# AvalonEnjoyer/pytorch-ViT-paper-replication

Hardware: AMD Instinct MI355X
Metric: images/sec (whole node) ViT-B/16 224px bf16 at 1/2/4/8 MI355X (higher is better)
Workload: dtype bf16; 1 GPU; model=ViT-B/16, global_batch=256, per_gpu_batch=256, seq_len=197, image_size=224, parallelism=dp1, impl=fused, grad_transport=none, optimizer=Adam(wd=0.03 decay group) + clip 1.0 + warmup/linear-decay LR, dropout=0.1 (mlp, embedding)

## Files before the change

### pytorch_vit_paper_replication_amd/csrc/bindings.cpp

```cpp
#include <cstdlib>
#include <algorithm>
#include <map>
#include <torch/extension.h>
#include <c10/hip/HIPStream.h>
#include <hip/hip_runtime.h>

#include "kernels.h"

namespace {

hipStream_t stream() { return c10::hip::getCurrentHIPStream().stream(); }
using ScratchKey = std::pair<int, int64_t>;
ScratchKey scratch_key(int dev) { return std::make_pair(dev, (int64_t)c10::hip::getCurrentHIPStream().id()); }
template <class T>
std::map<ScratchKey, T>& scratch_map() {
  static auto* m = new std::map<ScratchKey, T>();
  return *m;
}
struct SkCounters { torch::Tensor t; };
struct DetWs { torch::Tensor t; };
struct DqWs { torch::Tensor t; };
struct AttnWs { torch::Tensor t; };

int num_cus() {
// ... 733 lines not shown
void attn_dbias_reduce(torch::Tensor part, int64_t B, int64_t H, torch::Tensor dbias) {
  TORCH_CHECK(dbias.is_cuda() && dbias.scalar_type() == torch::kFloat32 && dbias.is_contiguous() && dbias.numel() % (3 * H) == 0,
              "attn_dbias_reduce: f32 [3D] bias gradient");
  const int64_t DH = dbias.numel() / (3 * H);
  TORCH_CHECK(part.is_cuda() && part.scalar_type() == torch::kFloat32 && part.is_contiguous() && part.numel() % (B * H * 3 * DH) == 0,
              "attn_dbias_reduce: f32 [B*H][R][3 * head dim] partials");
  const int64_t NQ = part.numel() / (B * H * 3 * DH);
  auto ws = torch::empty({(int64_t)pvr_attn_dbias_splits((int)B, (int)NQ) * H * 2 * DH}, part.options());
  check(pvr_attn_dbias_reduce(part.data_ptr<float>(), ws.data_ptr<float>(), dbias.data_ptr<float>(), (int)B, (int)H, (int)NQ,
                              (int)(DH * H), stream()),
        "attn_dbias_reduce");
}

torch::Tensor dq_workspace(int64_t numel, const torch::TensorOptions& opts, bool drop = false) {
  DqWs& d = scratch_map<DqWs>()[scratch_key((int)opts.device().index())];
  if (drop) {
    d.t = torch::Tensor();
    return torch::Tensor();
  }
  if (!d.t.defined() || d.t.numel() < numel) d.t = torch::zeros({numel}, opts.dtype(torch::kFloat32));
  return d.t;
}

torch::Tensor attn_scratch(int64_t numel, const torch::TensorOptions& opts) {
  AttnWs& d = scratch_map<AttnWs>()[scratch_key((int)opts.device().index())];
  if (!d.t.defined() || d.t.numel() < numel) d.t = torch::empty({numel}, opts.dtype(torch::kFloat32));
  return d.t;
}

void free_scratch() {
  scratch_map<TailBufs>().clear();
  scratch_map<SkCounters>().clear();
  scratch_map<DetWs>().clear();
  scratch_map<DqWs>().clear();
  scratch_map<AttnWs>().clear();
}

int64_t attn_bwd_bias_rows(int64_t B, int64_t N, int64_t H, int64_t D, bool drop) {
  return pvr_attn_bwd_part_rows((int)B, (int)N, (int)H, (int)D, 3 * D, D, D, 3 * D, drop ? 1 : 0);
}

bool attn_bwd_q8_ok(int64_t B, int64_t N, int64_t H, int64_t D, bool drop) {
  return pvr_attn_bwd_q8_ok((int)N, drop ? 1 : 0) && !pvr_attn_bwd_uses_pipe((int)B, (int)N, (int)H, (int)D, 3 * D, D, D, 3 * D, drop ? 1 : 0);
}

torch::Tensor attn_bwd(torch::Tensor dout, torch::Tensor qkv, torch::Tensor out, torch::Tensor lse, int64_t B, int64_t N, int64_t H,
                       double scale, c10::optional<torch::Tensor> dbias, c10::optional<torch::Tensor> dbias_part_out,
                       c10::optional<torch::Tensor> seed, int64_t seed_offset, double drop_p, c10::optional<torch::Tensor> q_out,
                       c10::optional<torch::Tensor> q_scale, c10::optional<torch::Tensor> q_amax, bool q_only,
                       int64_t q_fmt) {
  const int64_t D = qkv.size(1) / 3;
  auto dqkv = torch::empty_like(qkv);
  torch::Tensor dq_acc;
  int dq_rezero = 0;
  const pvr::DropSite drop = drop_args(seed, seed_offset, drop_p, "attn_bwd");
  const int has_drop = drop.seed ? 1 : 0;
  const int64_t dh = D / H;
  torch::Tensor dbias_part, old_part;
  const bool want_db = dbias.has_value() && dbias->defined();
  const int64_t lds[4] = {ld_of(qkv, "qkv"), ld_of(dout, "dout"), ld_of(out, "out"), ld_of(dqkv, "dqkv")};
  const int prow = pvr_attn_bwd_part_rows((int)B, (int)N, (int)H, (int)D, lds[0], lds[1], lds[2], lds[3], has_drop);
  const bool parts = prow > 0;
  const bool pipe = pvr_attn_bwd_uses_pipe((int)B, (int)N, (int)H, (int)D, lds[0], lds[1], lds[2], lds[3], has_drop) != 0;
  const bool part_out = dbias_part_out.has_value() && dbias_part_out->defined();
  if (part_out) {
    TORCH_CHECK(parts && !want_db, "dbias_part: shapes with attn_bwd_bias_rows > 0 only, and not together with dbias");
    TORCH_CHECK(dbias_part_out->is_cuda() && dbias_part_out->scalar_type() == torch::kFloat32 && dbias_part_out->is_contiguous() &&
                    dbias_part_out->numel() == B * H * prow * 3 * dh,
                "dbias_part [B*H][attn_bwd_bias_rows][3 * head dim] f32");
    dbias_part = *dbias_part_out;
  }
  if (want_db) {
    TORCH_CHECK(dbias->numel() == 3 * D && dbias->scalar_type() == torch::kFloat32 && dbias->is_contiguous(), "dbias [3D] f32");
    if (parts)
      dbias_part = torch::empty({B * H, (int64_t)prow, 3 * dh}, qkv.options().dtype(torch::kFloat32));
    else if (2 * (dh / 16) <= 2 * pvr_attn_bwd_waves((int)N))
      old_part = torch::empty({B * pvr_attn_bwd_key_blocks((int)N), 3 * D}, qkv.options().dtype(torch::kFloat32));
  }
  const int old_db = old_part.defined() ? 1 : 0;
  if (pvr_attn_bwd_needs_dq_acc((int)N, (int)dh, old_db, has_drop, g_deterministic ? 1 : 0)) {
    dq_acc = dq_workspace(B * N * D, qkv.options());
    dq_rezero = dq_acc.defined() ? 1 : 0;
    if (!dq_acc.defined()) dq_acc = torch::zeros({B * N, D}, qkv.options().dtype(torch::kFloat32));
  }
  const pvr::Fp8Copy q8 = fp8_copy(q_out, q_scale, q_amax, q_fmt, B * N, 3 * D, 4, "attn_bwd");
  if (q8.out)
    TORCH_CHECK(pvr_attn_bwd_q8_ok((int)N, has_drop) && !old_db && !pipe, "attn_bwd: no e5m2 dQKV copy for this shape (see attn_bwd_q8_ok)");
  auto ws = attn_scratch(pvr_attn_bwd_ws_floats((int)B, (int)N, (int)H, (int)D, old_db, has_drop, g_deterministic ? 1 : 0), qkv.options());
  pvr::AttnBwdParams p{};
  p.qkv = bf(qkv, "qkv"); p.ld = lds[0];
  p.out = bf(out, "out"); p.ld_o = lds[2];
  p.dout = bf(dout, "dout"); p.ld_do = lds[1];
  p.dqkv = bf_mut(dqkv, "dqkv"); p.ld_dq = lds[3];
  p.lse = f32(lse, "lse"); p.ws = ws.data_ptr<float>();
  p.dq_acc = dq_acc.defined() ? dq_acc.data_ptr<float>() : nullptr; p.dq_rezero = dq_rezero;
  p.dbias = pipe && dbias_part.defined() ? dbias_part.data_ptr<float>() : old_db ? old_part.data_ptr<float>() : nullptr;
  p.bpart = !pipe && dbias_part.defined() ? dbias_part.data_ptr<float>() : nullptr;
  p.B = (int)B; p.N = (int)N; p.H = (int)H; p.D = (int)D; p.scale = (float)scale;
  p.drop = drop; p.q8 = q8; p.q8_only = q_only && q8.out ? 1 : 0;
  const hipError_t err = pvr_attn_bwd(&p, stream());
  if (err != hipSuccess && dq_rezero) dq_workspace(0, qkv.options(), true);
  check(err, "attn_bwd");
  if (want_db) {
    if (parts)
      attn_dbias_reduce(dbias_part, B, H, *dbias);
    else if (old_db)
      dbias->add_(old_part.sum(0));
    else
      dbias->add_(dqkv.sum(0, false, torch::kFloat32));
  }
  return dqkv;
}

}

extern "C" const char* pvr_src_hash(void);

PYBIND11_MODULE(TORCH_EXTENSION_NAME, m) {
  m.doc() = "MI355X (gfx950) HIP kernels for pytorch_vit_paper_replication_amd";
  m.def("source_hash", []() { return std::string(pvr_src_hash()); },
        "content hash of the csrc/ sources this binary was built from (build.source_hash())");
  m.def("gemm_tail_split", [](int64_t M, int64_t N, int64_t K, int64_t elem_bytes, int64_t max_units) {
    return pvr_gemm_tail_split((int)M, (int)N, (int)K, (int)elem_bytes, (int)max_units); },
    py::arg("M"), py::arg("N"), py::arg("K"), py::arg("elem_bytes"), py::arg("max_units") = 0,
    "K-parts of the split tail round this GEMM shape gets (0: none)");
  m.def("set_attn_dbg", [](torch::Tensor t) { pvr_set_attn_dbg(t.defined() && t.numel() ? t.data_ptr() : nullptr); },
        "diagnostic builds (-DPVR_ATTN_STAMPS): int64 buffer for the attention backward's phase stamps "
        "[workgroup * waves + wave][8] (scripts/attn_stamps.py); a no-op otherwise");
  m.def("set_attn_prep_xcd", &pvr_set_attn_prep_xcd, "attention backward pre-pass: XCD-contiguous (batch, head) pairs (1) or round-robin (0, default); A/B");
  m.def("set_ln_fwd_q8_grid", &pvr_set_ln_fwd_q8_grid, "LayerNorm forward with the e4m3 copy: grid cap in workgroups per CU (A/B)");
  m.def("set_attn_fwd_head_qf", &pvr_set_attn_fwd_head_qf, "whole-head attention forward (dh 64, N <= 256): 16-query fragments per wave (1 = default, 2 = half the LDS reads with 7 waves; A/B)");
  m.def("set_attn_fwd_qg", &pvr_set_attn_fwd_qg, "tiled attention forward: 16-query groups per wave (0 = auto by query padding, 1 = round-3 form, 2 = forced; A/B)");
  m.def("set_fp8_persistent", &pvr_set_fp8_persistent, "fp8 fwd/dgrad GEMMs on the persistent ping-pong: 1 when the epilogue has no per-row input (default), 0 never (A/B)");
  m.def("set_deterministic", &set_deterministic, "deterministic reductions (partial rows + ordered sum) instead of float atomics");
  m.def("deterministic", &deterministic);
  m.def("set_gemm_tail", &set_gemm_tail, "split-K tail of the last dispatch round on (True, default) / off (A/B)");
  m.def("gemm", &gemm,py::arg("A"), py::arg("a_kcontig"), py::arg("B"), py::arg("b_kcontig"), py::arg("C"),
        py::arg("M"), py::arg("N"), py::arg("K"), py::arg("epi"), py::arg("bias"), py::arg("resid"), py::arg("addend"),
        py::arg("addend_period"), py::arg("aux"), py::arg("row_group"), py::arg("row_stride_group"),
        py::arg("row_offset"), py::arg("seed"), py::arg("seed_offset"), py::arg("drop_p"), py::arg("k_split"),
        py::arg("tile_cfg"), py::arg("dbg") = py::none(), py::arg("colsum") = py::none(),
        py::arg("epi_staged") = 0, py::arg("tail_limit") = 0, py::arg("reduce_out") = py::none(), py::arg("reduce_acc") = true);
  m.def("splitk_timeouts", &splitk_timeouts, py::arg("like"), py::arg("reset") = false);
  m.def("num_cus", &num_cus);
  m.def("layernorm_fwd", &layernorm_fwd);
  m.def("free_scratch", &free_scratch);
  m.def("layernorm_fwd_q8", &layernorm_fwd_q8);
  m.def("layernorm_bwd", &layernorm_bwd, py::arg("dy"), py::arg("dy_stride"), py::arg("x"), py::arg("x_stride"),
        py::arg("mean"), py::arg("rstd"), py::arg("w"), py::arg("dres"), py::arg("dres_stride"), py::arg("dx"),
        py::arg("dx_stride"), py::arg("dw"), py::arg("db"), py::arg("rows"), py::arg("dsum") = py::none(),
        py::arg("dz") = py::none(), py::arg("seed") = py::none(), py::arg("seed_offset") = 0, py::arg("drop_p") = 0.0,
        py::arg("q_out") = py::none(), py::arg("q_scale") = py::none(), py::arg("q_amax") = py::none(),
        py::arg("dz_nostore") = false, py::arg("q_fmt") = 1);
  m.def("cast_f32_bf16", &cast_f32_bf16);
  m.def("splitk_epilogue", &splitk_epilogue);
  m.def("attn_bwd_bias_rows", &attn_bwd_bias_rows, py::arg("B"), py::arg("N"), py::arg("H"), py::arg("D"), py::arg("drop") = false);
  m.def("attn_dbias_reduce", &attn_dbias_reduce);
  m.def("splitk_reduce", &splitk_reduce);
  m.def("pad_cols_bf16", &pad_cols_bf16);
  m.def("transpose_batched", &transpose_batched);
  m.def("colsum", &colsum, py::arg("dy"), py::arg("rows"), py::arg("N"), py::arg("db"), py::arg("dz"), py::arg("seed"),
        py::arg("seed_offset"), py::arg("drop_p"), py::arg("q_out") = py::none(), py::arg("q_scale") = py::none(),
        py::arg("q_amax") = py::none(), py::arg("q_fmt") = 1);
  m.def("im2col", &im2col);
  m.def("im2col_u8", &im2col_u8, py::arg("img"), py::arg("out"), py::arg("mean"), py::arg("std"), py::arg("geom"), py::arg("H"),
        py::arg("W"), py::arg("P"), py::arg("Kp"));
  m.def("cls_rows", &cls_rows);
  m.def("patch_bwd", &patch_bwd);
  m.def("xent", &xent, py::arg("logits"), py::arg("labels"), py::arg("dlogits"), py::arg("correct"), py::arg("grad_scale"),
        py::arg("mean") = py::none());
  m.def("grad_norm", &grad_norm);
  m.def("norm_partial_blocks", []() { return pvr_norm_partial_blocks(); });
  m.def("adam", &adam);
  m.def("adam_t", &adam_t);
  m.def("scale_by_clip", &scale_by_clip);
  m.def("head_fwd", &head_fwd);
  m.def("head_bwd", &head_bwd, py::arg("dlogits"), py::arg("xhat"), py::arg("rstd"), py::arg("gamma"), py::arg("beta"), py::arg("W"),
        py::arg("B"), py::arg("N"), py::arg("dW") = py::none(), py::arg("db") = py::none(), py::arg("dgamma") = py::none(),
        py::arg("dbeta") = py::none());
  m.def("scale_by", &scale_by);
  m.def("metrics_accum", &metrics_accum);
  m.def("rng_next", &rng_next);
  m.def("zero_f32", &zero_f32);
  m.def("gemm_fp8", &gemm_fp8, py::arg("A"), py::arg("fmt_a"), py::arg("B"), py::arg("fmt_b"), py::arg("C"), py::arg("M"),
        py::arg("N"), py::arg("K"), py::arg("epi"), py::arg("scale_a"), py::arg("scale_b"), py::arg("bias") = py::none(),
        py::arg("resid") = py::none(), py::arg("aux") = py::none(), py::arg("seed") = py::none(), py::arg("seed_offset") = 0,
        py::arg("drop_p") = 0.0, py::arg("colsum") = py::none(), py::arg("q_out") = py::none(), py::arg("q_scale") = py::none(),
        py::arg("q_amax") = py::none(), py::arg("q_fmt") = 0, py::arg("c_skip") = false, py::arg("tail_limit") = 0);
  m.def("fp8_transpose", &fp8_transpose);
  m.def("gemm_fp8_wgrad_mn", &gemm_fp8_wgrad_mn, py::arg("dy8"), py::arg("x8"), py::arg("ws"), py::arg("N"), py::arg("K"),
        py::arg("T"), py::arg("scale_a"), py::arg("scale_b"), py::arg("ksplit"), py::arg("fmt_a") = 1);
  m.def("fp8_quant", &fp8_quant, py::arg("x"), py::arg("y"), py::arg("qscale"), py::arg("amax"), py::arg("fmt"));
  m.def("fp8_dequant", &fp8_dequant, py::arg("x"), py::arg("dscale") = py::none(), py::arg("fmt") = 0);
  m.def("fp8_scale_update", &fp8_scale_update);
  m.def("fp8_quant_t", &fp8_quant_t);
  m.def("gemm_fp8_wgrad", &gemm_fp8_wgrad, py::arg("A8"), py::arg("B8"), py::arg("ws"), py::arg("N"), py::arg("K"), py::arg("Tp"),
        py::arg("scale_a"), py::arg("scale_b"), py::arg("ksplit"), py::arg("fmt_a") = 1);
  m.def("fp8_quant_multi", &fp8_quant_multi, py::arg("segs"), py::arg("nchunks"), py::arg("qscale"), py::arg("amax"), py::arg("fmt"),
        py::arg("amax_only"));
  m.def("attn_fwd", &attn_fwd, py::arg("qkv"), py::arg("B"), py::arg("N"), py::arg("H"), py::arg("scale"),
        py::arg("seed") = py::none(), py::arg("seed_offset") = 0, py::arg("drop_p") = 0.0, py::arg("q_out") = py::none(),
        py::arg("q_scale") = py::none(), py::arg("q_amax") = py::none(), py::arg("q_only") = false);
  m.def("attn_bwd", &attn_bwd, py::arg("dout"), py::arg("qkv"), py::arg("out"), py::arg("lse"), py::arg("B"), py::arg("N"),
        py::arg("H"), py::arg("scale"), py::arg("dbias") = py::none(), py::arg("dbias_part") = py::none(),
        py::arg("seed") = py::none(), py::arg("seed_offset") = 0, py::arg("drop_p") = 0.0, py::arg("q_out") = py::none(),
        py::arg("q_scale") = py::none(), py::arg("q_amax") = py::none(), py::arg("q_only") = false,
        py::arg("q_fmt") = 1);
  m.def("attn_bwd_q8_ok", &attn_bwd_q8_ok, "attn_bwd can write dQKV's e5m2 copy for this shape");
  m.def("arch", []() { return std::string("gfx950"); });
}
```

### pytorch_vit_paper_replication_amd/csrc/layernorm.hip

```cpp
#include "common.h"
#include "kernels.h"

namespace pvr {
namespace {

template <int MAXCH>
__global__ void __launch_bounds__(256) ln_fwd_kernel(const uint16_t* __restrict__ x, int64_t x_stride,
                                                      const float* __restrict__ w, const float* __restrict__ b,
                                                      uint16_t* __restrict__ y, int64_t y_stride,
                                                      float* __restrict__ mean_out, float* __restrict__ rstd_out,
                                                      int rows, int D, float eps) {
  const int lane = threadIdx.x & 63;
  const int row = blockIdx.x * 4 + (threadIdx.x >> 6);
  if (row >= rows) return;
  const int nch = D >> 3;
  PVR_ASSERT((D & 7) == 0 && nch <= 64 * MAXCH);
  const uint16_t* xr = x + (int64_t)row * x_stride;
  float v[MAXCH][8];
  float s = 0.f;
#pragma unroll
  for (int i = 0; i < MAXCH; ++i) {
    const int c = lane + 64 * i;
    if (c < nch) {
      const uint4 q = *(const uint4*)(xr + c * 8);
      const uint32_t u[4] = {q.x, q.y, q.z, q.w};
#pragma unroll
      for (int j = 0; j < 4; ++j) {
        v[i][2 * j] = bf2f(u[j] & 0xFFFF);
        v[i][2 * j + 1] = bf2f(u[j] >> 16);
      }
#pragma unroll
      for (int j = 0; j < 8; ++j) s += v[i][j];
    } else {
#pragma unroll
      for (int j = 0; j < 8; ++j) v[i][j] = 0.f;
    }
  }
  const float mean = wave_sum(s) / D;
  float ss = 0.f;
#pragma unroll
  for (int i = 0; i < MAXCH; ++i) {
    const int c = lane + 64 * i;
    if (c < nch) {
#pragma unroll
      for (int j = 0; j < 8; ++j) {
        const float d = v[i][j] - mean;
        ss += d * d;
      }
    }
  }
  const float rstd = rsqrtf(wave_sum(ss) / D + eps);
  uint16_t* yr = y + (int64_t)row * y_stride;
#pragma unroll
  for (int i = 0; i < MAXCH; ++i) {
    const int c = lane + 64 * i;
    if (c < nch) {
      const float4 w0 = *(const float4*)(w + c * 8), w1 = *(const float4*)(w + c * 8 + 4);
      const float4 b0 = *(const float4*)(b + c * 8), b1 = *(const float4*)(b + c * 8 + 4);
      const float ww[8] = {w0.x, w0.y, w0.z, w0.w, w1.x, w1.y, w1.z, w1.w};
      const float bb[8] = {b0.x, b0.y, b0.z, b0.w, b1.x, b1.y, b1.z, b1.w};
      float o[8];
#pragma unroll
      for (int j = 0; j < 8; ++j) o[j] = (v[i][j] - mean) * rstd * ww[j] + bb[j];
      uint4 q;
      q.x = pack2bf(o[0], o[1]); q.y = pack2bf(o[2], o[3]);
      q.z = pack2bf(o[4], o[5]); q.w = pack2bf(o[6], o[7]);
      *(uint4*)(yr + c * 8) = q;
    }
  }
  if (lane == 0) {
    mean_out[row] = mean;
    rstd_out[row] = rstd;
  }
}

template <int MAXCH>
__global__ void __launch_bounds__(256) ln_fwd_q8_kernel(const uint16_t* __restrict__ x, int64_t x_stride,
                                                        const float* __restrict__ w, const float* __restrict__ b,
                                                        uint16_t* __restrict__ y, int64_t y_stride, uint8_t* __restrict__ yq,
                                                        int64_t q_stride, const float* __restrict__ qscale,
                                                        unsigned* __restrict__ amax, float* __restrict__ mean_out,
                                                        float* __restrict__ rstd_out, int rows, int D, float eps) {
  __shared__ float wm[4];
  const int lane = threadIdx.x & 63;
  const int nch = D >> 3;
  const float qs = *qscale;
  float am = 0.f;
  for (int row = blockIdx.x * 4 + (int)(threadIdx.x >> 6); row < rows; row += gridDim.x * 4) {
    const uint16_t* xr = x + (int64_t)row * x_stride;
    float v[MAXCH][8];
    float s = 0.f;
#pragma unroll
    for (int i = 0; i < MAXCH; ++i) {
      const int c = lane + 64 * i;
      if (c < nch) {
        const uint4 q = *(const uint4*)(xr + c * 8);
        const uint32_t u[4] = {q.x, q.y, q.z, q.w};
#pragma unroll
        for (int j = 0; j < 4; ++j) {
          v[i][2 * j] = bf2f(u[j] & 0xFFFF);
          v[i][2 * j + 1] = bf2f(u[j] >> 16);
        }
#pragma unroll
        for (int j = 0; j < 8; ++j) s += v[i][j];
      } else {
#pragma unroll
        for (int j = 0; j < 8; ++j) v[i][j] = 0.f;
      }
    }
    const float mean = wave_sum(s) / D;
    float ss = 0.f;
#pragma unroll
    for (int i = 0; i < MAXCH; ++i) {
      const int c = lane + 64 * i;
      if (c < nch) {
#pragma unroll
        for (int j = 0; j < 8; ++j) {
          const float d = v[i][j] - mean;
          ss += d * d;
        }
      }
    }
    const float rstd = rsqrtf(wave_sum(ss) / D + eps);
    uint16_t* yr = y ? y + (int64_t)row * y_stride : nullptr;
    uint8_t* qr = yq + (int64_t)row * q_stride;
#pragma unroll
    for (int i = 0; i < MAXCH; ++i) {
      const int c = lane + 64 * i;
      if (c < nch) {
        const float4 w0 = *(const float4*)(w + c * 8), w1 = *(const float4*)(w + c * 8 + 4);
        const float4 b0 = *(const float4*)(b + c * 8), b1 = *(const float4*)(b + c * 8 + 4);
        const float ww[8] = {w0.x, w0.y, w0.z, w0.w, w1.x, w1.y, w1.z, w1.w};
        const float bb[8] = {b0.x, b0.y, b0.z, b0.w, b1.x, b1.y, b1.z, b1.w};
        float o[8];
        float vm = 0.f;
#pragma unroll
        for (int j = 0; j < 8; ++j) {
          o[j] = (v[i][j] - mean) * rstd * ww[j] + bb[j];
          vm = nan_max(vm, fabsf(o[j]));
        }
        am = nan_max(am, vm);
        uint4 q;
        q.x = pack2bf(o[0], o[1]); q.y = pack2bf(o[2], o[3]);
        q.z = pack2bf(o[4], o[5]); q.w = pack2bf(o[6], o[7]);
        if (yr) *(uint4*)(yr + c * 8) = q;
        *(uint2*)(qr + c * 8) = pack8_fp8_fast<0>(o, qs, vm);
      }
    }
    if (lane == 0) {
      mean_out[row] = mean;
      rstd_out[row] = rstd;
    }
  }
  am = wave_max_nan(am);
  if (lane == 0) wm[threadIdx.x >> 6] = am;
  __syncthreads();
  if (threadIdx.x == 0) {
    const float m = nan_max(nan_max(wm[0], wm[1]), nan_max(wm[2], wm[3]));
    if (!(m <= 0.f)) atomicMax(amax, __float_as_uint(m));
  }
}

PVR_DEV void load8(const uint16_t* p, float* o) {
  const uint4 q = *(const uint4*)p;
  const uint32_t u[4] = {q.x, q.y, q.z, q.w};
#pragma unroll
  for (int j = 0; j < 4; ++j) {
    o[2 * j] = bf2f(u[j] & 0xFFFF);
    o[2 * j + 1] = bf2f(u[j] >> 16);
  }
}

template <int W>
struct RowVec;
template <>
struct RowVec<8> {
  uint32_t u[4];
  PVR_DEV void load(const uint16_t* p) { const uint4 q = *(const uint4*)p; u[0] = q.x; u[1] = q.y; u[2] = q.z; u[3] = q.w; }
  PVR_DEV void store(uint16_t* p) const { *(uint4*)p = make_uint4(u[0], u[1], u[2], u[3]); }
  PVR_DEV void zero() { u[0] = u[1] = u[2] = u[3] = 0u; }
};
template <>
struct RowVec<4> {
  uint32_t u[2];
  PVR_DEV void load(const uint16_t* p) { const uint2 q = *(const uint2*)p; u[0] = q.x; u[1] = q.y; }
  PVR_DEV void store(uint16_t* p) const { *(uint2*)p = make_uint2(u[0], u[1]); }
  PVR_DEV void zero() { u[0] = u[1] = 0u; }
};

template <int MAXCH, int W, bool Q8>
__global__ void __launch_bounds__(256) ln_bwd_kernel(const uint16_t* __restrict__ dy, int64_t dy_stride,
                                                      const uint16_t* __restrict__ x, int64_t x_stride,
                                                      const float* __restrict__ mean, const float* __restrict__ rstd,
                                                      const float* __restrict__ w,
                                                      const uint16_t* __restrict__ dres, int64_t dres_stride,
                                                      uint16_t* __restrict__ dx, int64_t dx_stride,
                                                      float* __restrict__ dw, float* __restrict__ db, float* __restrict__ dsum,
                                                      float* __restrict__ part,
                                                      uint16_t* __restrict__ dz, int64_t dz_stride,
                                                      const uint64_t* __restrict__ seed_ptr, uint64_t seed_off, uint32_t thr,
                                                      float dscale, int dz_nostore, uint8_t* __restrict__ qout, int64_t q_stride,
                                                      const float* __restrict__ qscale, unsigned* __restrict__ amax, int qfmt,
                                                      int rows, int D) {
  __shared__ float red[4][MAXCH * 64 * W > 1280 ? 1280 : MAXCH * 64 * W];
  __shared__ float qred[4];
  const float qs = Q8 ? *qscale : 1.f;
  float qam = 0.f;
  const int lane = threadIdx.x & 63, wave = threadIdx.x >> 6;
  const int nch = D / W;
  float gw[MAXCH][W], gb[MAXCH][W], gs[MAXCH][W];
#pragma unroll
  for (int i = 0; i < MAXCH; ++i)
#pragma unroll
    for (int j = 0; j < W; ++j) gw[i][j] = gb[i][j] = gs[i][j] = 0.f;

  const int stride = gridDim.x * 4;
  RowVec<W> cx[MAXCH], cdy[MAXCH], cr[MAXCH];
  auto load_row = [&](int row, RowVec<W> (&qx)[MAXCH], RowVec<W> (&qd)[MAXCH], RowVec<W> (&qr)[MAXCH]) {
    const int rr = min(row, rows - 1);
#pragma unroll
    for (int i = 0; i < MAXCH; ++i) {
      const int c = min(lane + 64 * i, nch - 1);
      qx[i].load(x + (int64_t)rr * x_stride + c * W);
      qd[i].load(dy + (int64_t)rr * dy_stride + c * W);
      if (dres)
        qr[i].load(dres + (int64_t)rr * dres_stride + c * W);
      else
        qr[i].zero();
    }
  };
  float wreg[MAXCH][W];
#pragma unroll
  for (int i = 0; i < MAXCH; ++i) {
    const int c = min(lane + 64 * i, nch - 1);
#pragma unroll
    for (int j = 0; j < W; j += 4) {
      const float4 w4 = *(const float4*)(w + c * W + j);
      wreg[i][j] = w4.x; wreg[i][j + 1] = w4.y; wreg[i][j + 2] = w4.z; wreg[i][j + 3] = w4.w;
    }
  }
  const uint64_t seed = dz ? *seed_ptr + seed_off : 0ull;
  int row = blockIdx.x * 4 + wave;
  load_row(row, cx, cdy, cr);
  float cmu = row < rows ? mean[row] : 0.f, crs = row < rows ? rstd[row] : 0.f;
  for (; row < rows; row += stride) {
    RowVec<W> nx[MAXCH], ndy[MAXCH], nr[MAXCH];
    load_row(row + stride, nx, ndy, nr);
    const int rn = min(row + stride, rows - 1);
    const float nmu = mean[rn], nrs = rstd[rn];
    const float mu = cmu, rs = crs;
    auto xhat = [&](int i, int j) { return (bf2f(j & 1 ? cx[i].u[j >> 1] >> 16 : cx[i].u[j >> 1] & 0xFFFF) - mu) * rs; };
    auto dyv = [&](int i, int j) { return bf2f(j & 1 ? cdy[i].u[j >> 1] >> 16 : cdy[i].u[j >> 1] & 0xFFFF); };
    float s1 = 0.f, s2 = 0.f;
#pragma unroll
    for (int i = 0; i < MAXCH; ++i) {
      const int c = lane + 64 * i;
      if (c < nch) {
#pragma unroll
        for (int j = 0; j < W; ++j) {
          const float xh = xhat(i, j), dv = dyv(i, j);
          const float g = dv * wreg[i][j];
          s1 += g;
          s2 += g * xh;
          gw[i][j] += dv * xh;
          gb[i][j] += dv;
        }
      }
    }
    const float c1 = wave_sum(s1) / D, c2 = wave_sum(s2) / D;
#pragma unroll
    for (int i = 0; i < MAXCH; ++i) {
      const int c = lane + 64 * i;
      if (c < nch) {
        float o[W];
#pragma unroll
        for (int j = 0; j < W; ++j) o[j] = (dyv(i, j) * wreg[i][j] - c1 - xhat(i, j) * c2) * rs;
        if (dres) {
#pragma unroll
          for (int j = 0; j < W; ++j) o[j] += bf2f(j & 1 ? cr[i].u[j >> 1] >> 16 : cr[i].u[j >> 1] & 0xFFFF);
        }
        RowVec<W> q;
#pragma unroll
        for (int j = 0; j < W; j += 2) q.u[j >> 1] = pack2bf(o[j], o[j + 1]);
        q.store(dx + (int64_t)row * dx_stride + c * W);
        if (dz) {
#pragma unroll
          for (int j = 0; j < W; j += 2) {
            bool k0, k1;
            rng_keep2(seed, (uint64_t)row * D + c * W + j, thr, k0, k1);
            o[j] = k0 ? o[j] * dscale : 0.f;
            o[j + 1] = k1 ? o[j + 1] * dscale : 0.f;
          }
          if (!Q8 || !dz_nostore) {
#pragma unroll
            for (int j = 0; j < W; j += 2) q.u[j >> 1] = pack2bf(o[j], o[j + 1]);
            q.store(dz + (int64_t)row * dz_stride + c * W);
          }
        }
        if constexpr (Q8) {
          uint32_t b4[W / 4];
          float vm = 0.f;
#pragma unroll
          for (int j = 0; j < W; ++j) vm = nan_max(vm, fabsf(o[j]));
          qam = nan_max(qam, vm);
          if (qfmt ? fp8_direct_ok<1>(vm, qs) : fp8_direct_ok<0>(vm, qs)) {
#pragma unroll
            for (int j = 0; j < W; j += 4)
              b4[j >> 2] = qfmt ? pack4_fp8_direct<1>(o[j] * qs, o[j + 1] * qs, o[j + 2] * qs, o[j + 3] * qs)
                                : pack4_fp8_direct<0>(o[j] * qs, o[j + 1] * qs, o[j + 2] * qs, o[j + 3] * qs);
          } else {
#pragma unroll
            for (int j = 0; j < W; j += 4) b4[j >> 2] = pack4_fp8_rt(qfmt, o[j] * qs, o[j + 1] * qs, o[j + 2] * qs, o[j + 3] * qs);
          }
          uint8_t* qp = qout + (int64_t)row * q_stride + c * W;
          if constexpr (W == 8)
            *(uint2*)qp = make_uint2(b4[0], b4[1]);
          else
            *(uint32_t*)qp = b4[0];
        }
#pragma unroll
        for (int j = 0; j < W; ++j) gs[i][j] += o[j];
      }
    }
#pragma unroll
    for (int i = 0; i < MAXCH; ++i) {
      cx[i] = nx[i];
      cdy[i] = ndy[i];
      cr[i] = nr[i];
    }
    cmu = nmu;
    crs = nrs;
  }
  float* outs[3] = {dw, db, dsum};
#pragma unroll
  for (int qn = 0; qn < 3; ++qn) {
    if (!outs[qn]) continue;
    if (qn) __syncthreads();
#pragma unroll
    for (int i = 0; i < MAXCH; ++i) {
      const int c = lane + 64 * i;
      if (c < nch) {
#pragma unroll
        for (int j = 0; j < W; ++j) red[wave][c * W + j] = qn == 0 ? gw[i][j] : (qn == 1 ? gb[i][j] : gs[i][j]);
      }
    }
    __syncthreads();
    if (part) {
      float* pr = part + ((int64_t)blockIdx.x * 3 + qn) * D;
      for (int col = threadIdx.x; col < D; col += 256) pr[col] = red[0][col] + red[1][col] + red[2][col] + red[3][col];
    } else {
      for (int col = threadIdx.x; col < D; col += 256)
        atomicAdd(outs[qn] + col, red[0][col] + red[1][col] + red[2][col] + red[3][col]);
    }
  }
  if constexpr (Q8) {
    qam = wave_max_nan(qam);
    if (lane == 0) qred[wave] = qam;
    __syncthreads();
    if (threadIdx.x == 0) {
      const float m = nan_max(nan_max(qred[0], qred[1]), nan_max(qred[2], qred[3]));
      if (!(m <= 0.f)) atomicMax(amax, __float_as_uint(m));
    }
  }
}

}
}

static int device_cus() {
  static const int n = [] {
    int dev = 0, cus = 0;
    if (hipGetDevice(&dev) != hipSuccess || hipDeviceGetAttribute(&cus, hipDeviceAttributeMultiprocessorCount, dev) != hipSuccess ||
        cus <= 0)
      cus = 256;
    return cus;
  }();
  return n;
}

extern "C" hipError_t pvr_layernorm_fwd(const uint16_t* x, int64_t x_stride, const float* w, const float* b,
                                        uint16_t* y, int64_t y_stride, float* mean, float* rstd, int rows, int D,
                                        float eps, hipStream_t s) {
  using namespace pvr;
  if (rows <= 0) return hipSuccess;
  if (D % 8 != 0 || D > 2048) return hipErrorInvalidValue;
  const dim3 grid((rows + 3) / 4), block(256);
  const int maxch = (D / 8 + 63) / 64;
  switch (maxch) {
    case 1: hipLaunchKernelGGL(ln_fwd_kernel<1>, grid, block, 0, s, x, x_stride, w, b, y, y_stride, mean, rstd, rows, D, eps); break;
    case 2: hipLaunchKernelGGL(ln_fwd_kernel<2>, grid, block, 0, s, x, x_stride, w, b, y, y_stride, mean, rstd, rows, D, eps); break;
    case 3: hipLaunchKernelGGL(ln_fwd_kernel<3>, grid, block, 0, s, x, x_stride, w, b, y, y_stride, mean, rstd, rows, D, eps); break;
    default: hipLaunchKernelGGL(ln_fwd_kernel<4>, grid, block, 0, s, x, x_stride, w, b, y, y_stride, mean, rstd, rows, D, eps); break;
  }
  return hipGetLastError();
}

static int g_ln_q8_blocks_per_cu = 4;
extern "C" void pvr_set_ln_fwd_q8_grid(int per_cu) { g_ln_q8_blocks_per_cu = per_cu < 1 ? 1 : per_cu > 64 ? 64 : per_cu; }

extern "C" hipError_t pvr_layernorm_fwd_q8(const uint16_t* x, int64_t x_stride, const float* w, const float* b, uint16_t* y,
                                           int64_t y_stride, pvr::Fp8Copy q, float* mean, float* rstd, int rows, int D, float eps,
                                           hipStream_t s) {
  using namespace pvr;
  if (rows <= 0) return hipSuccess;
  if (D % 8 != 0 || D > 2048 || q.ld % 8 != 0) return hipErrorInvalidValue;
  int nblk = (rows + 3) / 4;
  const int cap = g_ln_q8_blocks_per_cu * device_cus();
  if (nblk > cap) nblk = cap;
  const dim3 grid(nblk), block(256);
  switch ((D / 8 + 63) / 64) {
    case 1: hipLaunchKernelGGL(ln_fwd_q8_kernel<1>, grid, block, 0, s, x, x_stride, w, b, y, y_stride, q.out, q.ld, q.scale, q.amax, mean, rstd, rows, D, eps); break;
    case 2: hipLaunchKernelGGL(ln_fwd_q8_kernel<2>, grid, block, 0, s, x, x_stride, w, b, y, y_stride, q.out, q.ld, q.scale, q.amax, mean, rstd, rows, D, eps); break;
    case 3: hipLaunchKernelGGL(ln_fwd_q8_kernel<3>, grid, block, 0, s, x, x_stride, w, b, y, y_stride, q.out, q.ld, q.scale, q.amax, mean, rstd, rows, D, eps); break;
    default: hipLaunchKernelGGL(ln_fwd_q8_kernel<4>, grid, block, 0, s, x, x_stride, w, b, y, y_stride, q.out, q.ld, q.scale, q.amax, mean, rstd, rows, D, eps); break;
  }
  return hipGetLastError();
}

extern "C" int pvr_layernorm_bwd_blocks(int rows, int D) {
  const bool use_w4 = (D / 4) % 64 == 0 && (D / 8) % 64 != 0 && D / 4 <= 64 * 5;
  const int cap = use_w4 && D == 768 ? device_cus() * 3 : 1024;
  const int nblk = (rows + 3) / 4;
  return nblk > cap ? cap : nblk;
}

extern "C" hipError_t pvr_layernorm_bwd(const pvr::LnBwdParams* pp, hipStream_t s) {
  using namespace pvr;
  const LnBwdParams& p = *pp;
  const DropSite& d = p.drop;
  const Fp8Copy& q = p.q;
  const int rows = p.rows, D = p.D;
  if (rows <= 0) return hipSuccess;
  if (q.fmt != 0 && q.fmt != 1) return hipErrorInvalidValue;
  if (D % 8 != 0 || D > 1280 || (p.dz && (!d.seed || !d.thr))) return hipErrorInvalidValue;
  if (q.out && (!q.scale || !q.amax || q.ld % 8 != 0 || reinterpret_cast<uintptr_t>(q.out) % 8 != 0)) return hipErrorInvalidValue;
  if (p.dz_nostore && (!p.dz || !q.out)) return hipErrorInvalidValue;
  const bool use_w4 = (D / 4) % 64 == 0 && (D / 8) % 64 != 0 && D / 4 <= 64 * 5;
  const int nblk = pvr_layernorm_bwd_blocks(rows, D);
  float* part = p.dw || p.db || p.dsum ? p.part : nullptr;
  const dim3 grid(nblk), block(256);
#define PVR_LN_BWD(MC, W)                                                                                                   \
  hipLaunchKernelGGL(q.out ? (ln_bwd_kernel<MC, W, true>) : (ln_bwd_kernel<MC, W, false>), grid, block, 0, s, p.dy, p.dy_stride, p.x, p.x_stride, p.mean, p.rstd, p.w, p.dres, p.dres_stride, p.dx, \
                     p.dx_stride, p.dw, p.db, p.dsum, part, p.dz, p.dz_stride, d.seed, d.offset, d.thr, d.scale, p.dz_nostore, q.out, q.ld, q.scale, q.amax, \
                     q.fmt, rows, D)
  if (use_w4) {
    switch (D / 256) {
      case 3: PVR_LN_BWD(3, 4); break;
      case 5: PVR_LN_BWD(5, 4); break;
      default: PVR_LN_BWD(1, 4); break;
    }
  } else {
    const int maxch = (D / 8 + 63) / 64;
    switch (maxch) {
      case 1: PVR_LN_BWD(1, 8); break;
      case 2: PVR_LN_BWD(2, 8); break;
      default: PVR_LN_BWD(3, 8); break;
    }
  }
#undef PVR_LN_BWD
  const hipError_t e = hipGetLastError();
  if (e != hipSuccess || !part) return e;
  return pvr_rows_reduce(part, nblk, 3 * D, D, p.dw, p.db, p.dsum, s);
}
```

Before: 7519 images/sec.

## Rewrite LayerNorm forward as persistent half-wave-per-row kernel with prefetch

Merges the plain and FP8 LayerNorm forward kernels into one template. For D=768 it maps 32 lanes to each row (two rows per wave), hoists gamma/beta into registers once per block, and uses a grid-stride persistent loop that prefetches the next row while the current one is processed. The grid is capped at a per-CU multiple. The aim is better memory-level parallelism and fewer redundant weight loads in this bandwidth-bound kernel, in exchange for more register pressure (MAXCH=3 of 8 floats each for x, w and b). It also exposes layernorm_bwd_blocks to Python.

```diff
diff --git a/pytorch_vit_paper_replication_amd/csrc/bindings.cpp b/pytorch_vit_paper_replication_amd/csrc/bindings.cpp
--- a/pytorch_vit_paper_replication_amd/csrc/bindings.cpp
+++ b/pytorch_vit_paper_replication_amd/csrc/bindings.cpp
@@ -909,6 +909,8 @@
         py::arg("dz") = py::none(), py::arg("seed") = py::none(), py::arg("seed_offset") = 0, py::arg("drop_p") = 0.0,
         py::arg("q_out") = py::none(), py::arg("q_scale") = py::none(), py::arg("q_amax") = py::none(),
         py::arg("dz_nostore") = false, py::arg("q_fmt") = 1);
+  m.def("layernorm_bwd_blocks", &pvr_layernorm_bwd_blocks, py::arg("rows"), py::arg("D"),
+        "workgroups of the layernorm_bwd grid (4 rows each per grid stride)");
   m.def("cast_f32_bf16", &cast_f32_bf16);
   m.def("splitk_epilogue", &splitk_epilogue);
   m.def("attn_bwd_bias_rows", &attn_bwd_bias_rows, py::arg("B"), py::arg("N"), py::arg("H"), py::arg("D"), py::arg("drop") = false);
diff --git a/pytorch_vit_paper_replication_amd/csrc/layernorm.hip b/pytorch_vit_paper_replication_amd/csrc/layernorm.hip
--- a/pytorch_vit_paper_replication_amd/csrc/layernorm.hip
+++ b/pytorch_vit_paper_replication_amd/csrc/layernorm.hip
@@ -3,173 +3,6 @@
 
 namespace pvr {
 namespace {
-
-template <int MAXCH>
-__global__ void __launch_bounds__(256) ln_fwd_kernel(const uint16_t* __restrict__ x, int64_t x_stride,
-                                                      const float* __restrict__ w, const float* __restrict__ b,
-                                                      uint16_t* __restrict__ y, int64_t y_stride,
-                                                      float* __restrict__ mean_out, float* __restrict__ rstd_out,
-                                                      int rows, int D, float eps) {
-  const int lane = threadIdx.x & 63;
-  const int row = blockIdx.x * 4 + (threadIdx.x >> 6);
-  if (row >= rows) return;
-  const int nch = D >> 3;
-  PVR_ASSERT((D & 7) == 0 && nch <= 64 * MAXCH);
-  const uint16_t* xr = x + (int64_t)row * x_stride;
-  float v[MAXCH][8];
-  float s = 0.f;
-#pragma unroll
-  for (int i = 0; i < MAXCH; ++i) {
-    const int c = lane + 64 * i;
-    if (c < nch) {
-      const uint4 q = *(const uint4*)(xr + c * 8);
-      const uint32_t u[4] = {q.x, q.y, q.z, q.w};
-#pragma unroll
-      for (int j = 0; j < 4; ++j) {
-        v[i][2 * j] = bf2f(u[j] & 0xFFFF);
-        v[i][2 * j + 1] = bf2f(u[j] >> 16);
-      }
-#pragma unroll
-      for (int j = 0; j < 8; ++j) s += v[i][j];
-    } else {
-#pragma unroll
-      for (int j = 0; j < 8; ++j) v[i][j] = 0.f;
-    }
-  }
-  const float mean = wave_sum(s) / D;
-  float ss = 0.f;
-#pragma unroll
-  for (int i = 0; i < MAXCH; ++i) {
-    const int c = lane + 64 * i;
-    if (c < nch) {
-#pragma unroll
-      for (int j = 0; j < 8; ++j) {
-        const float d = v[i][j] - mean;
-        ss += d * d;
-      }
-    }
-  }
-  const float rstd = rsqrtf(wave_sum(ss) / D + eps);
-  uint16_t* yr = y + (int64_t)row * y_stride;
-#pragma unroll
-  for (int i = 0; i < MAXCH; ++i) {
-    const int c = lane + 64 * i;
-    if (c < nch) {
-      const float4 w0 = *(const float4*)(w + c * 8), w1 = *(const float4*)(w + c * 8 + 4);
-      const float4 b0 = *(const float4*)(b + c * 8), b1 = *(const float4*)(b + c * 8 + 4);
-      const float ww[8] = {w0.x, w0.y, w0.z, w0.w, w1.x, w1.y, w1.z, w1.w};
-      const float bb[8] = {b0.x, b0.y, b0.z, b0.w, b1.x, b1.y, b1.z, b1.w};
-      float o[8];
-#pragma unroll
-      for (int j = 0; j < 8; ++j) o[j] = (v[i][j] - mean) * rstd * ww[j] + bb[j];
-      uint4 q;
-      q.x = pack2bf(o[0], o[1]); q.y = pack2bf(o[2], o[3]);
-      q.z = pack2bf(o[4], o[5]); q.w = pack2bf(o[6], o[7]);
-      *(uint4*)(yr + c * 8) = q;
-    }
-  }
-  if (lane == 0) {
-    mean_out[row] = mean;
-    rstd_out[row] = rstd;
-  }
-}
-
-template <int MAXCH>
-__global__ void __launch_bounds__(256) ln_fwd_q8_kernel(const uint16_t* __restrict__ x, int64_t x_stride,
-                                                        const float* __restrict__ w, const float* __restrict__ b,
-                                                        uint16_t* __restrict__ y, int64_t y_stride, uint8_t* __restrict__ yq,
-                                                        int64_t q_stride, const float* __restrict__ qscale,
-                                                        unsigned* __restrict__ amax, float* __restrict__ mean_out,
-                                                        float* __restrict__ rstd_out, int rows, int D, float eps) {
-  __shared__ float wm[4];
-  const int lane = threadIdx.x & 63;
-  const int nch = D >> 3;
-  const float qs = *qscale;
-  float am = 0.f;
-  for (int row = blockIdx.x * 4 + (int)(threadIdx.x >> 6); row < rows; row += gridDim.x * 4) {
-    const uint16_t* xr = x + (int64_t)row * x_stride;
-    float v[MAXCH][8];
-    float s = 0.f;
-#pragma unroll
-    for (int i = 0; i < MAXCH; ++i) {
-      const int c = lane + 64 * i;
-      if (c < nch) {
-        const uint4 q = *(const uint4*)(xr + c * 8);
-        const uint32_t u[4] = {q.x, q.y, q.z, q.w};
-#pragma unroll
-        for (int j = 0; j < 4; ++j) {
-          v[i][2 * j] = bf2f(u[j] & 0xFFFF);
-          v[i][2 * j + 1] = bf2f(u[j] >> 16);
-        }
-#pragma unroll
-        for (int j = 0; j < 8; ++j) s += v[i][j];
-      } else {
-#pragma unroll
-        for (int j = 0; j < 8; ++j) v[i][j] = 0.f;
-      }
-    }
-    const float mean = wave_sum(s) / D;
-    float ss = 0.f;
-#pragma unroll
-    for (int i = 0; i < MAXCH; ++i) {
-      const int c = lane + 64 * i;
-      if (c < nch) {
-#pragma unroll
-        for (int j = 0; j < 8; ++j) {
-          const float d = v[i][j] - mean;
-          ss += d * d;
-        }
-      }
-    }
-    const float rstd = rsqrtf(wave_sum(ss) / D + eps);
-    uint16_t* yr = y ? y + (int64_t)row * y_stride : nullptr;
-    uint8_t* qr = yq + (int64_t)row * q_stride;
-#pragma unroll
-    for (int i = 0; i < MAXCH; ++i) {
-      const int c = lane + 64 * i;
-      if (c < nch) {
-        const float4 w0 = *(const float4*)(w + c * 8), w1 = *(const float4*)(w + c * 8 + 4);
-        const float4 b0 = *(const float4*)(b + c * 8), b1 = *(const float4*)(b + c * 8 + 4);
-        const float ww[8] = {w0.x, w0.y, w0.z, w0.w, w1.x, w1.y, w1.z, w1.w};
-        const float bb[8] = {b0.x, b0.y, b0.z, b0.w, b1.x, b1.y, b1.z, b1.w};
-        float o[8];
-        float vm = 0.f;
-#pragma unroll
-        for (int j = 0; j < 8; ++j) {
-          o[j] = (v[i][j] - mean) * rstd * ww[j] + bb[j];
-          vm = nan_max(vm, fabsf(o[j]));
-        }
-        am = nan_max(am, vm);
-        uint4 q;
-        q.x = pack2bf(o[0], o[1]); q.y = pack2bf(o[2], o[3]);
-        q.z = pack2bf(o[4], o[5]); q.w = pack2bf(o[6], o[7]);
-        if (yr) *(uint4*)(yr + c * 8) = q;
-        *(uint2*)(qr + c * 8) = pack8_fp8_fast<0>(o, qs, vm);
-      }
-    }
-    if (lane == 0) {
-      mean_out[row] = mean;
-      rstd_out[row] = rstd;
-    }
-  }
-  am = wave_max_nan(am);
-  if (lane == 0) wm[threadIdx.x >> 6] = am;
-  __syncthreads();
-  if (threadIdx.x == 0) {
-    const float m = nan_max(nan_max(wm[0], wm[1]), nan_max(wm[2], wm[3]));
-    if (!(m <= 0.f)) atomicMax(amax, __float_as_uint(m));
-  }
-}
-
-PVR_DEV void load8(const uint16_t* p, float* o) {
-  const uint4 q = *(const uint4*)p;
-  const uint32_t u[4] = {q.x, q.y, q.z, q.w};
-#pragma unroll
-  for (int j = 0; j < 4; ++j) {
-    o[2 * j] = bf2f(u[j] & 0xFFFF);
-    o[2 * j + 1] = bf2f(u[j] >> 16);
-  }
-}
 
 template <int W>
 struct RowVec;
@@ -187,6 +20,131 @@
   PVR_DEV void store(uint16_t* p) const { *(uint2*)p = make_uint2(u[0], u[1]); }
   PVR_DEV void zero() { u[0] = u[1] = 0u; }
 };
+
+template <int LPR>
+PVR_DEV float row_sum(float v) {
+  if constexpr (LPR == 64) {
+    return wave_sum(v);
+  } else {
+    v = row16_sum(v);
+    return v + __shfl_xor(v, 16);
+  }
+}
+
+template <int MAXCH, int LPR, bool Q8>
+__global__ void __launch_bounds__(256) ln_fwd_kernel(const uint16_t* __restrict__ x, int64_t x_stride,
+                                                      const float* __restrict__ w, const float* __restrict__ b,
+                                                      uint16_t* __restrict__ y, int64_t y_stride, uint8_t* __restrict__ yq,
+                                                      int64_t q_stride, const float* __restrict__ qscale,
+                                                      unsigned* __restrict__ amax, float* __restrict__ mean_out,
+                                                      float* __restrict__ rstd_out, int rows, int D, float eps) {
+  constexpr int RPW = 64 / LPR;
+  __shared__ float wm[4];
+  const float qs = Q8 ? *qscale : 1.f;
+  float am = 0.f;
+  const int lane = threadIdx.x & 63;
+  const int rl = lane & (LPR - 1), sub = lane / LPR;
+  const int nch = D >> 3;
+  PVR_ASSERT((D & 7) == 0 && nch <= LPR * MAXCH);
+  float wreg[MAXCH][8], breg[MAXCH][8];
+#pragma unroll
+  for (int i = 0; i < MAXCH; ++i) {
+    const int c = min(rl + LPR * i, nch - 1);
+    const float4 w0 = *(const float4*)(w + c * 8), w1 = *(const float4*)(w + c * 8 + 4);
+    const float4 b0 = *(const float4*)(b + c * 8), b1 = *(const float4*)(b + c * 8 + 4);
+    wreg[i][0] = w0.x; wreg[i][1] = w0.y; wreg[i][2] = w0.z; wreg[i][3] = w0.w;
+    wreg[i][4] = w1.x; wreg[i][5] = w1.y; wreg[i][6] = w1.z; wreg[i][7] = w1.w;
+    breg[i][0] = b0.x; breg[i][1] = b0.y; breg[i][2] = b0.z; breg[i][3] = b0.w;
+    breg[i][4] = b1.x; breg[i][5] = b1.y; breg[i][6] = b1.z; breg[i][7] = b1.w;
+  }
+  auto load_row = [&](int64_t row, RowVec<8> (&q)[MAXCH]) {
+    const int64_t rr = row < rows ? row : rows - 1;
+#pragma unroll
+    for (int i = 0; i < MAXCH; ++i) q[i].load(x + rr * x_stride + min(rl + LPR * i, nch - 1) * 8);
+  };
+  const int64_t stride = (int64_t)gridDim.x * 4 * RPW;
+  int64_t row = ((int64_t)blockIdx.x * 4 + (threadIdx.x >> 6)) * RPW + sub;
+  RowVec<8> cx[MAXCH];
+  load_row(row, cx);
+  for (int64_t r0 = row - sub; r0 < rows; r0 += stride, row += stride) {
+    RowVec<8> nx[MAXCH];
+    load_row(row + stride, nx);
+    float v[MAXCH][8];
+    float s = 0.f;
+#pragma unroll
+    for (int i = 0; i < MAXCH; ++i) {
+      const bool on = rl + LPR * i < nch;
+#pragma unroll
+      for (int j = 0; j < 4; ++j) {
+        v[i][2 * j] = on ? bf2f(cx[i].u[j] & 0xFFFF) : 0.f;
+        v[i][2 * j + 1] = on ? bf2f(cx[i].u[j] >> 16) : 0.f;
+      }
+#pragma unroll
+      for (int j = 0; j < 8; ++j) s += v[i][j];
+    }
+    const float mean = row_sum<LPR>(s) / D;
+    float ss = 0.f;
+#pragma unroll
+    for (int i = 0; i < MAXCH; ++i) {
+      if (rl + LPR * i < nch) {
+#pragma unroll
+        for (int j = 0; j < 8; ++j) {
+          const float d = v[i][j] - mean;
+          ss += d * d;
+        }
+      }
+    }
+    const float rstd = rsqrtf(row_sum<LPR>(ss) / D + eps);
+    if (row < rows) {
+      uint16_t* yr = y ? y + row * y_stride : nullptr;
+#pragma unroll
+      for (int i = 0; i < MAXCH; ++i) {
+        const int c = rl + LPR * i;
+        if (c < nch) {
+          float o[8];
+#pragma unroll
+          for (int j = 0; j < 8; ++j) o[j] = (v[i][j] - mean) * rstd * wreg[i][j] + breg[i][j];
+          RowVec<8> q;
+#pragma unroll
+          for (int j = 0; j < 4; ++j) q.u[j] = pack2bf(o[2 * j], o[2 * j + 1]);
+          if (!Q8 || yr) q.store(yr + c * 8);
+          if constexpr (Q8) {
+            float vm = 0.f;
+#pragma unroll
+            for (int j = 0; j < 8; ++j) vm = nan_max(vm, fabsf(o[j]));
+            am = nan_max(am, vm);
+            *(uint2*)(yq + row * q_stride + c * 8) = pack8_fp8_fast<0>(o, qs, vm);
+          }
+        }
+      }
+      if (rl == 0) {
+        mean_out[row] = mean;
+        rstd_out[row] = rstd;
+      }
+    }
+#pragma unroll
+    for (int i = 0; i < MAXCH; ++i) cx[i] = nx[i];
+  }
+  if constexpr (Q8) {
+    am = wave_max_nan(am);
+    if (lane == 0) wm[threadIdx.x >> 6] = am;
+    __syncthreads();
+    if (threadIdx.x == 0) {
+      const float m = nan_max(nan_max(wm[0], wm[1]), nan_max(wm[2], wm[3]));
+      if (!(m <= 0.f)) atomicMax(amax, __float_as_uint(m));
+    }
+  }
+}
+
+PVR_DEV void load8(const uint16_t* p, float* o) {
+  const uint4 q = *(const uint4*)p;
+  const uint32_t u[4] = {q.x, q.y, q.z, q.w};
+#pragma unroll
+  for (int j = 0; j < 4; ++j) {
+    o[2 * j] = bf2f(u[j] & 0xFFFF);
+    o[2 * j + 1] = bf2f(u[j] >> 16);
+  }
+}
 
 template <int MAXCH, int W, bool Q8>
 __global__ void __launch_bounds__(256) ln_bwd_kernel(const uint16_t* __restrict__ dy, int64_t dy_stride,
@@ -378,21 +336,45 @@
   return n;
 }
 
+static hipError_t ln_fwd_launch(const uint16_t* x, int64_t x_stride, const float* w, const float* b, uint16_t* y, int64_t y_stride,
+                                const pvr::Fp8Copy& q, float* mean, float* rstd, int rows, int D, float eps, int blocks_per_cu,
+                                hipStream_t s) {
+  using namespace pvr;
+  const int nch = D / 8;
+  const bool half = nch <= 32 || (nch % 32 == 0 && nch % 64 != 0 && nch <= 32 * 5);
+  const int per_block = half ? 8 : 4;
+  const int maxch = half ? (nch + 31) / 32 : (nch + 63) / 64;
+  const int cap = (blocks_per_cu > 0 ? blocks_per_cu : (maxch <= 3 ? 16 : 8)) * device_cus();
+  int nblk = (rows + per_block - 1) / per_block;
+  if (nblk > cap) nblk = cap;
+  const dim3 grid(nblk), block(256);
+#define PVR_LN_FWD(MC, LPR)                                                                                                  \
+  hipLaunchKernelGGL(q.out ? (ln_fwd_kernel<MC, LPR, true>) : (ln_fwd_kernel<MC, LPR, false>), grid, block, 0, s, x, x_stride, w, b, y, \
+                     y_stride, q.out, q.ld, q.scale, q.amax, mean, rstd, rows, D, eps)
+  if (half) {
+    switch (maxch) {
+      case 1: PVR_LN_FWD(1, 32); break;
+      case 3: PVR_LN_FWD(3, 32); break;
+      default: PVR_LN_FWD(5, 32); break;
+    }
+  } else {
+    switch (maxch) {
+      case 1: PVR_LN_FWD(1, 64); break;
+      case 2: PVR_LN_FWD(2, 64); break;
+      case 3: PVR_LN_FWD(3, 64); break;
+      default: PVR_LN_FWD(4, 64); break;
+    }
+  }
+#undef PVR_LN_FWD
+  return hipGetLastError();
+}
+
 extern "C" hipError_t pvr_layernorm_fwd(const uint16_t* x, int64_t x_stride, const float* w, const float* b,
                                         uint16_t* y, int64_t y_stride, float* mean, float* rstd, int rows, int D,
                                         float eps, hipStream_t s) {
-  using namespace pvr;
   if (rows <= 0) return hipSuccess;
-  if (D % 8 != 0 || D > 2048) return hipErrorInvalidValue;
-  const dim3 grid((rows + 3) / 4), block(256);
-  const int maxch = (D / 8 + 63) / 64;
-  switch (maxch) {
-    case 1: hipLaunchKernelGGL(ln_fwd_kernel<1>, grid, block, 0, s, x, x_stride, w, b, y, y_stride, mean, rstd, rows, D, eps); break;
-    case 2: hipLaunchKernelGGL(ln_fwd_kernel<2>, grid, block, 0, s, x, x_stride, w, b, y, y_stride, mean, rstd, rows, D, eps); break;
-    case 3: hipLaunchKernelGGL(ln_fwd_kernel<3>, grid, block, 0, s, x, x_stride, w, b, y, y_stride, mean, rstd, rows, D, eps); break;
-    default: hipLaunchKernelGGL(ln_fwd_kernel<4>, grid, block, 0, s, x, x_stride, w, b, y, y_stride, mean, rstd, rows, D, eps); break;
-  }
-  return hipGetLastError();
+  if (D % 8 != 0 || D > 2048 || !y) return hipErrorInvalidValue;
+  return ln_fwd_launch(x, x_stride, w, b, y, y_stride, pvr::Fp8Copy{}, mean, rstd, rows, D, eps, 0, s);
 }
 
 static int g_ln_q8_blocks_per_cu = 4;
@@ -401,20 +383,9 @@
 extern "C" hipError_t pvr_layernorm_fwd_q8(const uint16_t* x, int64_t x_stride, const float* w, const float* b, uint16_t* y,
                                            int64_t y_stride, pvr::Fp8Copy q, float* mean, float* rstd, int rows, int D, float eps,
                                            hipStream_t s) {
-  using namespace pvr;
   if (rows <= 0) return hipSuccess;
-  if (D % 8 != 0 || D > 2048 || q.ld % 8 != 0) return hipErrorInvalidValue;
-  int nblk = (rows + 3) / 4;
-  const int cap = g_ln_q8_blocks_per_cu * device_cus();
-  if (nblk > cap) nblk = cap;
-  const dim3 grid(nblk), block(256);
-  switch ((D / 8 + 63) / 64) {
-    case 1: hipLaunchKernelGGL(ln_fwd_q8_kernel<1>, grid, block, 0, s, x, x_stride, w, b, y, y_stride, q.out, q.ld, q.scale, q.amax, mean, rstd, rows, D, eps); break;
-    case 2: hipLaunchKernelGGL(ln_fwd_q8_kernel<2>, grid, block, 0, s, x, x_stride, w, b, y, y_stride, q.out, q.ld, q.scale, q.amax, mean, rstd, rows, D, eps); break;
-    case 3: hipLaunchKernelGGL(ln_fwd_q8_kernel<3>, grid, block, 0, s, x, x_stride, w, b, y, y_stride, q.out, q.ld, q.scale, q.amax, mean, rstd, rows, D, eps); break;
-    default: hipLaunchKernelGGL(ln_fwd_q8_kernel<4>, grid, block, 0, s, x, x_stride, w, b, y, y_stride, q.out, q.ld, q.scale, q.amax, mean, rstd, rows, D, eps); break;
-  }
-  return hipGetLastError();
+  if (D % 8 != 0 || D > 2048 || q.ld % 8 != 0 || !q.out || !q.scale || !q.amax) return hipErrorInvalidValue;
+  return ln_fwd_launch(x, x_stride, w, b, y, y_stride, q, mean, rstd, rows, D, eps, g_ln_q8_blocks_per_cu, s);
 }
 
 extern "C" int pvr_layernorm_bwd_blocks(int rows, int D) {
```

Result: no change. 7550 images/sec, median of 6 (+0.4%).
